# paulvoliva/XNODE-WAN-PDE-solver

Hardware: AMD Instinct MI355X
Metric: WAN training-steps/sec (optimiser sub-steps, d=20 cube, N_r=4096 paths per GPU) (higher is better)
Workload: dtype f64

## Files before the change

### include/xnwan.h

```cpp
#ifndef XNWAN_H
#define XNWAN_H
#ifdef __cplusplus
extern "C" {
#endif

#define XW_E_DIMS     (-1)
#define XW_E_ARG      (-2)
#define XW_E_WORKSPACE (-3)
#define XW_E_COMM     (-4)

int xw_abi_version(void);
int xw_supported_dims(char* buf, int buflen);

int xw_theta_size(int d, int H, int K);
int xw_phi_size(int d, int W);

int xw_ode_fwd(const double* xT, const double* t, const double* start, const double* theta,
               int method, int N, int L, int d, int H, int K, int m,
               double* u, double* Y, void* stream);

typedef struct { const double* xT; const double* start; double* u; double* Y; double* act; int N;
                 int act_x_only;
                 int narrow;
                 int prio_drop;
// ... 120 lines not shown
int xw_slab_sum(const double* gslab, int nslab, int P, int accumulate, double* out, void* stream);
int xw_slab_sum2(const double* gA, int nA, double* outA, const double* gB, int nB, double* outB, int P, void* stream);

typedef struct {
  int N, Nb, L, Lb, d;
  int same_grid;
  int w_per_point, amode, pair_i, pair_b;
  int ns_u, ns_b;
  int narrow;
  int sharded;
  double Vol, Nglob, Nbglob, s3_scale, init_off, bdry_off, ckappa;
  const double *xT, *xvT, *xbT, *t, *tb, *tpp, *xvT_pts;
  const double *start, *start_b, *h, *href, *f, *g, *w, *wt, *w0, *ghT, *gwx0T, *c, *cp, *A0, *B0;
  double *u, *ub, *Y, *Yb, *act, *act_b, *v, *vt, *gxv, *gtv, *gx, *gs, *vbar, *s3x, *vact, *slabA, *slabB, *slab_v, *work_i, *work_b;
  double *xproj;
} XwGroup;
typedef int (*XwExchangeFn)(double* buf, int count, void* ctx, void* stream);
typedef struct {
  int method, H, K, m, W, q, Pu, Pv, adjoint;
  int v_blocks, v_blocks_disc;
  int lag_lo, lag_hi;
  double alpha, pollution, lr_u, lr_v, beta1, beta2, eps;
  double *theta, *phi, *scal, *grad_u, *grad_v, *m_u, *v_u, *m_v, *v_v;
  long long *step_u, *step_v, *lag_u;
  XwExchangeFn exchange;
  void* exchange_ctx;
  double* pack_u;
  int merged_sweep;
} XwSolverState;
int xw_substep_gen(const XwGroup* g, const XwSolverState* s, int skip_v, int store_record, double* accum, int adam_skip_field,
// ... 27 lines not shown
```

### xnode_wan_pde_solver_amd/_lib.py

```python
import ctypes
import os

_HERE = os.path.dirname(os.path.abspath(__file__))
LIB_PATH = os.environ.get('XW_LIBRARY') or os.path.join(_HERE, 'libxnwan.so')
ABI_VERSION = 33

c_f32p = ctypes.c_void_p
c_f64p = ctypes.c_void_p
c_i64p = ctypes.c_void_p
c_int, c_dbl, c_vp = ctypes.c_int, ctypes.c_double, ctypes.c_void_p


class XwOdeFwdJob(ctypes.Structure):
    _fields_ = [('xT', c_vp), ('start', c_vp), ('u', c_vp), ('Y', c_vp), ('act', c_vp), ('N', c_int), ('act_x_only', c_int),
                ('narrow', c_int), ('prio_drop', c_int)]


class XwOdeBwdJob(ctypes.Structure):
    _fields_ = [('xT', c_vp), ('start', c_vp), ('Y', c_vp), ('act', c_vp), ('ubar', c_vp), ('gx', c_vp), ('gs', c_vp),
                ('gslab', c_vp), ('N', c_int), ('res_first_only', c_int), ('res_u', c_vp), ('res_ref', c_vp),
                ('res_coef', ctypes.c_double), ('res_base', ctypes.c_double), ('res_w_per_point', c_int), ('res_w', c_vp),
                ('res_c', c_vp), ('res_cp', c_vp), ('res_kappa2', ctypes.c_double), ('res_scal', c_vp), ('res_refA', c_vp),
                ('res_coefA', ctypes.c_double), ('res_baseA', ctypes.c_double)]

# ... 7 lines not shown
    _fields_ = [('xT', c_vp), ('start', c_vp), ('u', c_vp), ('Y', c_vp), ('rec_y', c_vp), ('rec_t', c_vp), ('rec_h', c_vp),
                ('fbuf', c_vp), ('ctl', c_vp), ('work', c_vp), ('N', c_int), ('cap', c_int)]


class XwDopriSweepJob(ctypes.Structure):
    _fields_ = [('b', XwOdeBwdJob), ('rec_y', c_vp), ('rec_t', c_vp), ('rec_h', c_vp), ('ctl', c_vp)]


class XwGroup(ctypes.Structure):
    _fields_ = ([(n, c_int) for n in ('N', 'Nb', 'L', 'Lb', 'd', 'same_grid', 'w_per_point', 'amode', 'pair_i', 'pair_b', 'ns_u', 'ns_b',
                                      'narrow', 'sharded')]
                + [(n, c_dbl) for n in ('Vol', 'Nglob', 'Nbglob', 's3_scale', 'init_off', 'bdry_off', 'ckappa')]
                + [(n, c_vp) for n in ('xT', 'xvT', 'xbT', 't', 'tb', 'tpp', 'xvT_pts', 'start', 'start_b', 'h', 'href', 'f', 'g', 'w',
                                       'wt', 'w0', 'ghT', 'gwx0T', 'c', 'cp', 'A0', 'B0', 'u', 'ub', 'Y', 'Yb', 'act', 'act_b', 'v',
                                       'vt', 'gxv', 'gtv', 'gx', 'gs', 'vbar', 's3x', 'vact', 'slabA', 'slabB', 'slab_v', 'work_i',
                                       'work_b', 'xproj')])


class XwSolverState(ctypes.Structure):
    _fields_ = ([(n, c_int) for n in ('method', 'H', 'K', 'm', 'W', 'q', 'Pu', 'Pv', 'adjoint', 'v_blocks', 'v_blocks_disc', 'lag_lo',
                                      'lag_hi')]
                + [(n, c_dbl) for n in ('alpha', 'pollution', 'lr_u', 'lr_v', 'beta1', 'beta2', 'eps')]
                + [(n, c_vp) for n in ('theta', 'phi', 'scal', 'grad_u', 'grad_v', 'm_u', 'v_u', 'm_v', 'v_v', 'step_u', 'step_v',
                                       'lag_u', 'exchange', 'exchange_ctx', 'pack_u')]
                + [('merged_sweep', c_int)])


EXCHANGE_FN = ctypes.CFUNCTYPE(ctypes.c_int, ctypes.c_void_p, ctypes.c_int, ctypes.c_void_p, ctypes.c_void_p)


SIGNATURES = {
# ... 124 lines not shown
```

### xnode_wan_pde_solver_amd/csrc/xw_disc.hip

```cpp
#include "xw_common.h"
#include "xw_generic.h"
#include <atomic>
#include <cstdlib>

namespace {

template <int W> struct VDim {
  static constexpr int MT = (W + 15) / 16;
  static constexpr int KS = (W + 3) / 4;
  static constexpr int TR = W - 16 * (MT - 1);
  static constexpr bool VTAIL = TR <= 3;
  static constexpr int MTF = VTAIL ? MT - 1 : MT;
  __device__ static constexpr int LR(int mt) { return (W + 1 - 16 * mt) >= 16 ? 4 : (W + 1 - 16 * mt + 3) / 4; }
  static constexpr bool BIASROW = (W % 16) != 0;
  static_assert(MT == 4 || MT == 6 || MT == 8, "row tiles of the compiled widths");
};

struct Pt {
  int p, n;
  bool valid;
  double t;
};
__device__ __forceinline__ Pt locate(long tile, long P, int N, const double* __restrict__ tf, const double* __restrict__ tpp) {
  Pt q;
// ... 106 lines not shown
  for (long it = (long)blockIdx.x * 4 + wave; it < ntiles;) {
    const long tile = DYN ? it : (it < G ? it - rot + (it < rot ? G : 0) : it);
    long nxt = it + G;
    unsigned int ticket = 0;
    if (DYN && lane == 0) ticket = atomicAdd(queue + cur * XW_DISC_QSTRIDE, 1u);
    const Pt pt = locate(tile, P, N, tf, tpp);
    const bool want_grad = gxv != nullptr && tile * 16 < ngrad;
    d4 a[D::MT], ad[D::MT];
    const long tu = __builtin_amdgcn_readfirstlane((int)tile);
    double* actl = act + tu * ((long)(q + 1) * W * 16);
    asm volatile("" : "+s"(actl));
    const int aoff = lane;
    const double* pht = ph;
    asm volatile("" : "+s"(pht));
    if (XPROJ) {
      const double* xp = xproj + pt.n;
#pragma unroll
      for (int mt = 0; mt < D::MT; ++mt)
#pragma unroll
        for (int r = 0; r < 4; ++r) {
          ad[mt][r] = sIn[16 * mt + g + 4 * r];
          a[mt][r] = (16 * mt + 4 * r < W) ? fma(ad[mt][r], pt.t, xw_ld_g(xp + (long)(16 * mt + 4 * r + g) * N)) : 0.0;
        }
    } else if (VINLDS) {
#pragma unroll
      for (int mt = 0; mt < D::MT; ++mt)
#pragma unroll
        for (int r = 0; r < 4; ++r) {
          ad[mt][r] = sIn[16 * mt + g + 4 * r];
          a[mt][r] = sIn[16 * D::MT + 16 * mt + g + 4 * r] + ad[mt][r] * pt.t;
        }
      for (int ks = 0; ks < ksl; ++ks) {
        const int i = 4 * ks + g;
        const double b = i < d ? xT[(long)i * N + pt.n] : 0.0;
#pragma unroll
        for (int mt = 0; mt < D::MT; ++mt) a[mt] = XW_MFMA(sVin[(ks * D::MT + mt) * 64 + lane], b, a[mt]);
      }
// ... 1129 lines not shown
```

### xnode_wan_pde_solver_amd/csrc/xw_substep.hip

```cpp
#include <hip/hip_runtime.h>
#include <string.h>
#include "xnwan.h"

namespace {
struct Side {
  hipStream_t s = nullptr;
  hipEvent_t fork = nullptr, fwd = nullptr, done = nullptr;
};
Side* side_of_current_device() {
  static Side sides[64];
  int dev = 0;
  if (hipGetDevice(&dev) != hipSuccess || dev < 0 || dev >= 64) return nullptr;
  Side& x = sides[dev];
  if (x.s == nullptr) {
    if (hipStreamCreateWithFlags(&x.s, hipStreamNonBlocking) != hipSuccess) return nullptr;
    if (hipEventCreateWithFlags(&x.fork, hipEventDisableTiming) != hipSuccess || hipEventCreateWithFlags(&x.fwd, hipEventDisableTiming) != hipSuccess ||
        hipEventCreateWithFlags(&x.done, hipEventDisableTiming) != hipSuccess)
      return nullptr;
  }
  return &x;
}
#define XW_HIP(call) { const hipError_t e_ = (call); if (e_ != hipSuccess) return (int)e_; }

inline XwOdeFwdJob fwd_job(const double* xT, const double* start, double* u, double* Y, double* act, int N, int x_only, int narrow) {
// ... 1 lines not shown
  j.xT = xT; j.start = start; j.u = u; j.Y = Y; j.act = act; j.N = N; j.act_x_only = x_only; j.narrow = narrow; j.prio_drop = 0;
  return j;
}
inline XwOdeBwdJob bwd_job(const double* xT, const double* start, const double* Y, const double* act, int N) {
  XwOdeBwdJob j;
  memset(&j, 0, sizeof(j));
  j.xT = xT; j.start = start; j.Y = Y; j.act = act; j.N = N;
  return j;
}
#define XW_TRY(call) { const int rc_ = (call); if (rc_ != 0) return rc_; }

int test_net(const XwGroup* g, const XwSolverState* s, int blocks, double* record, void* stream) {
  if (g->tpp != nullptr)
    return xw_disc_fwd(g->xvT_pts, nullptr, g->tpp, s->phi, g->N * g->L, 1, g->d, s->W, s->q, g->v, g->vt, g->gxv, g->gtv, g->N, blocks,
                       record, stream);
  if (g->xproj != nullptr) XW_TRY(xw_disc_xproj(g->xvT, s->phi, g->N, g->d, s->W, g->xproj, stream));
  return xw_disc_fwd_xproj(g->xvT, g->t, nullptr, s->phi, g->N, g->L, g->d, s->W, s->q, g->v, g->vt, g->gxv, g->gtv, g->N, blocks, record,
                           g->xproj, stream);
}
int contract(const XwGroup* g, const XwSolverState* s, long long* step, bool with_bdry, bool finalize, void* stream) {
  const double* s3x = nullptr;
  if (g->A0 != nullptr || g->B0 != nullptr) {
    XW_TRY(xw_weak_contract_general(g->A0, g->amode, g->B0, g->gx, g->gs, g->ghT, g->gxv, g->w0, g->gwx0T, g->v, g->d, g->N, g->s3x,
                                    stream));
    s3x = g->s3x;
  }
  const bool fused = s3x == nullptr;
  return xw_weak_partials(g->u, g->v, g->vt, g->w, g->w_per_point, g->wt, s3x, fused ? g->gx : nullptr, fused ? g->gs : nullptr,
                          fused ? g->ghT : nullptr, fused ? g->gxv : nullptr, fused ? g->w0 : nullptr, fused ? g->gwx0T : nullptr,
                          fused ? g->d : 0, g->c, g->ckappa, g->f, g->h, g->pair_i ? g->href : nullptr, g->pair_i ? 1 : 0,
                          g->pair_i ? g->s3_scale : 1.0, g->N, g->L, g->Vol, g->Nglob, g->work_i, s->scal, finalize ? 1 : 0,
// ... 189 lines not shown
      XW_TRY(xw_disc_bwd(g->xvT_pts, nullptr, g->tpp, s->phi, g->vbar, g->N * g->L, 1, g->d, s->W, s->q, record, g->slab_v, stream));
    } else {
      XW_TRY(xw_disc_bwd(g->xvT, g->t, nullptr, s->phi, g->vbar, g->N, g->L, g->d, s->W, s->q, record, g->slab_v, stream));
    }
  }
  if (!shard) {
    XW_TRY(xw_adam(s->phi, g->slab_v, nsv, accum, nullptr, 0, nullptr, nullptr, s->m_v, s->v_v, s->step_v, -1, s->Pv, s->lr_v, s->beta1,
                   s->beta2, s->eps, s->grad_v, 0, 0, 0, nullptr, stream));
  } else {
    if (have_i) { XW_TRY(xw_slab_sum(g->slab_v, nsv, s->Pv, 0, s->grad_v, stream)); } else { XW_ZERO(s->grad_v, s->Pv); }
    XW_TRY(s->exchange(s->grad_v, s->Pv, s->exchange_ctx, stream));
    XW_TRY(xw_losses(s->scal, g->L, g->Lb > 0 ? g->Lb : 1, g->Vol, g->Nglob, g->Nbglob, s->alpha, 0.0, 0.0, s->step_v, stream));
    XW_TRY(xw_adam(s->phi, accum, accum != nullptr ? 1 : 0, s->grad_v, nullptr, 0, nullptr, nullptr, s->m_v, s->v_v, s->step_v, -1, s->Pv,
                   s->lr_v, s->beta1, s->beta2, s->eps, s->grad_v, 0, 0, 0, nullptr, stream));
  }
  if (accum != nullptr) {
    const hipError_t e = hipMemcpyAsync(accum, s->grad_v, sizeof(double) * s->Pv, hipMemcpyDeviceToDevice, (hipStream_t)stream);
    if (e != hipSuccess) return (int)e;
  }
  return 0;
}
```

### xnode_wan_pde_solver_amd/engine.py

```python
import contextlib
import math
import os

import torch

from . import kernels as KN
from ._lib import XnwanError
from .options import EngineOptions
from .sampling import HIP_HOST_LOCK, _PIN_POOL, Hypercube, _paths


def ctypes_addr(fn):
    import ctypes
    return ctypes.cast(fn, ctypes.c_void_p).value

_KEPT_GRAPHS = []

_NOSTREAM = contextlib.nullcontext()

_SCRATCH_POOL = []


_DEVICE_STREAMS = {}

# ... 126 lines not shown
                                                                              KN.GENERIC_ODE_MAX_DEPTH, sorted(KN.METHODS)))
        self.testnet = getattr(v_mod, 'family', None) or KN.testnet_family(config['v_hidden_dim'], self.q)
        self.testnet_tiled = self.testnet == 'tiled'
        if self.testnet_tiled and self.W != config['v_hidden_dim']:
            raise XnwanError('the tiled test-network family reads phi at the network\'s own width; the module was bound at %d' % self.W)
        self.generic = (self.stepper == 'generic', not self.testnet_tiled and KN.disc_generic(self.W))
        if any(self.generic):
            import warnings
            which = ' and '.join(n_ for n_, g_ in zip(('u_theta (u_hidden_dim %d, u_hidden_hidden_dim %d, u_layers %d)' % (self.H, self.K, self.m),
                                                       'v_phi (v_hidden_dim %d)' % self.W), self.generic) if g_)
            warnings.warn('%s is outside the MFMA kernel instantiations %s (u_layers <= 10) / %s: running on the generic vector-ALU path, expect a step '
                          'rate lower by two to three orders of magnitude' % (which, KN.ODE_WIDTHS, KN.DISC_WIDTHS), RuntimeWarning, stacklevel=3)
        self.xproj_min_d = 1 << 30 if (self.generic[1] or self.testnet_tiled) else int(opt.xproj_min_d)
        if self.W > 64 and not self.generic[1] and not self.testnet_tiled:
            self.xproj_min_d = 0
        if self.generic[0] and self.adjoint:
            raise XnwanError('adjoint=True (the continuous adjoint) exists for the MFMA stepper instantiations %s only; u_hidden_dim = %d, '
                             'u_hidden_hidden_dim = %d run on the generic path, which reverses the steps taken (adjoint=False)'
                             % (KN.ODE_WIDTHS, self.H, self.K))
        self.theta, self.phi = u_mod.blob, v_mod.blob
        self.Pu, self.Pv = self.theta.data.numel(), self.phi.data.numel()
        z = lambda n: torch.zeros(n, dtype=F64, device=device)
        self.adam_u = dict(m=z(self.Pu), v=z(self.Pu), step=torch.zeros(1, dtype=torch.int64, device=device),
                           lag=torch.zeros(1, dtype=torch.int64, device=device))
        self.pairwise_single_slice = opt.pairwise_single_slice
        self.adam_skips_untouched = opt.adam_skips_untouched
        self.eager_checked = 10 ** 12 if opt.always_check else 256
        self.field_range = (self.theta.slots[6][0], self.theta.slots[-2][0])
        self._field_touched = False
        self.adam_v = dict(m=z(self.Pv), v=z(self.Pv), step=torch.zeros(1, dtype=torch.int64, device=device))
# ... 308 lines not shown
        pair_state = dict(pair_i=pair_i, pair_b=pair_b, init_off=init_off, bdry_off=bdry_off, s3_scale=nglob if pair_i else 1.0,
                          sharded=sharded, has_bdry=BX is not None and (nb_glob if sharded else Nb) > 0)
        if into is not None:
            G = into
            same = (G.N, G.L, G.Nb, G.Lb, G.same_grid, G.Vol, G.Nglob, G.Nbglob, G.pair_i, G.pair_b, G.amode, G.sharded) == (
                N, L, Nb, Lb, same_grid, vol, nglob, nbglob, pair_i, pair_b, amode, sharded) and all(
                (getattr(G, k) is None) == (S[k] is None) and (S[k] is None or getattr(G, k).shape == S[k].shape)
                for k in Group.SAMPLE_FIELDS)
            if same:
                for k in Group.SAMPLE_FIELDS:
                    if S[k] is not None:
                        getattr(G, k).copy_(S[k])
                G.domain = domain
                G.__dict__.update(pair_state)
                G.sample_version += 1
                return G
        G = Group()
        for k in Group.SAMPLE_FIELDS:
            setattr(G, k, S[k])
        G.domain, G.N, G.L, G.Nb, G.Vol, G.Nglob, G.Nbglob = domain, N, L, Nb, vol, nglob, nbglob
        G.Lb, G.same_grid, G.amode = Lb, same_grid, amode
        G.__dict__.update(pair_state)
        self._work_buffers(G, [])
        G.graphs = {}
        G.sample_version = into.sample_version + 1 if into is not None else 0
        return G

    def load_groups_packed(self, shards, hints, domain, cache, big):
        tc = getattr(self, '_tab_cat', None)
        st = self.structure
        if (tc is None or not (st.a_identity and st.b_zero and st.c_kappa is not None)
                or getattr(domain, 'time_independent', False) or any(h is None for h in hints)):
            return None
        srcs = [tc[k] for k in ('f', 'g', 'w', 'gw', 'start', 'gh', 'h', 'start_b')]
        if any(t.dtype != F64 or not t.is_cuda for t in srcs) or any(t.dtype != F64 or not t.is_cuda or t_[0] is not t_[1]
                                                                       for t_ in shards for t in t_[:3]):
            return None
        d, dev, T0 = self.d, self.dev, self.setup['T0']
        f_cat, g_cat, w_cat, gw_cat, start, gh, hv, sb = srcs
        if f_cat.stride(0) != 1 or g_cat.stride(0) != 1 or w_cat.stride(0) != 1:
# ... 6 lines not shown
        for k, ((X, XV, BX, n_glob, nb_glob, grids), hn) in enumerate(zip(shards, hints)):
            N, L, Nb, Lb = X.shape[0], X.shape[1], BX.shape[0], BX.shape[1]
            sharded = n_glob is not None and self.world is not None
            shared = bool(hn['shared_times'])
            same_grid = Lb == L and bool(hn['same_grid'])
            starts_T0, b_T0 = bool(tc['at0'][k]), bool(tc['bat0'][k])
            G = Group()
            G.domain, G.N, G.L, G.Nb, G.Vol = domain, N, L, Nb, vol
            G.Nglob, G.Nbglob = float(n_glob if n_glob is not None else N), float(nb_glob if nb_glob is not None else max(Nb, 1))
            G.Lb, G.same_grid, G.amode = Lb, same_grid, 0
            fields = [('t', (L,)), ('xT', (d, N))]
            if not shared:
                fields += [('tpp', (L * N,)), ('tpp0', (N,)), ('xvT_pts', (d, L * N))]
            fields += [('start', (N,)), ('ghT', (d, N)), ('h', (N,)), ('f', (L, N)), ('w', (L, N)), ('wt', (L, N)), ('w0', (N,)), ('gwx0T', (d, N)),
                       ('tb', (Lb,)), ('xbT', (d, Nb)), ('start_b', (Nb,)), ('g', (Lb, Nb))]
            self._work_buffers(G, fields)
            G._lazy['xvT'] = G._lazy['xT']
            if shared:
                G.tpp = G.tpp0 = G.xvT_pts = None
            G.href = G.X = G.A0 = G.B0 = None
            base = G._arena.data_ptr()
            x0, x1, x2 = X.stride()
            b0, b1, b2 = BX.stride()
            xp, bp = X.data_ptr(), BX.data_ptr()
            t_src = (xp, x1) if grids is None else (grids[0].data_ptr(), grids[0].stride(0))
            tb_src = (bp, b1) if grids is None else (grids[1].data_ptr(), grids[1].stride(0))
            src = {'t': (t_src[0], 1, 1, L, 0, 0, t_src[1]), 'xT': (xp + 8 * x2, 1, d, N, 0, x2, x0),
                   'tpp': (xp, 1, L, N, 0, x1, x0), 'tpp0': (xp, 1, 1, N, 0, 0, x0), 'xvT_pts': (xp + 8 * x2, d, L, N, x2, 0, x0),
                   'start': (start.data_ptr() + 8 * oN * start.stride(0), 1, 1, N, 0, 0, start.stride(0)),
                   'ghT': (gh.data_ptr() + 8 * oN * h0, 1, d, N, 0, h1, h0),
                   'h': (hv.data_ptr() + 8 * oN * hv.stride(0), 1, 1, N, 0, 0, hv.stride(0)),
# ... 22 lines not shown
            G.sample_version = ver + 1 if old is not None else 0
            if self.verify_structure and k == big and ver % self.verify_every == 0:
                self._check_structure(X, ver // self.verify_every)
            groups.append(G)
            oN, oNL, oNb, oNbL = oN + N, oNL + N * L, oNb + Nb, oNbL + Nb * Lb
        if len(rows) > KN.GATHER_ROWS:
            return None
        table = torch.zeros(KN.GATHER_ROWS, 9, dtype=torch.int64)
        table[:len(rows)] = torch.tensor(rows, dtype=torch.int64)
        from .sampling import _PIN_POOL
        pinned = _PIN_POOL.stage(table)
        tdev = pinned.to(dev, non_blocking=True)
        _PIN_POOL.uploaded(pinned, torch.cuda.current_stream(dev))
        KN.gather_fields(tdev, len(rows), total)
        for G in groups:
            if G.pair_i and not st.b_zero:
                raise XnwanError('func_b != 0 on a single-slice group at T0 (see load_group)')
            if G.pair_i or G.pair_b:
                zero = torch.zeros((), dtype=F64, device=dev)
                gsum, gsq = (G.g.sum(), (G.g ** 2).sum()) if G.pair_b else (zero, zero)
                stats = torch.stack([G.h.sum(), (G.h ** 2).sum(), G.f.sum(), gsum, gsq]).contiguous()
                if G.sharded:
                    self.world.all_reduce(stats)
                sh, shh, sf, sg, sgg = stats.tolist()
                if G.pair_i:
                    G.href = torch.full((G.N,), sh / G.Nglob, dtype=F64, device=dev)
                    G.f.fill_(sf / G.Nglob)
                    G.init_off = shh / G.Nglob - (sh / G.Nglob) ** 2
                if G.pair_b:
                    G.g.fill_(sg / G.Nbglob)
                    G.bdry_off = sgg / G.Nbglob - (sg / G.Nbglob) ** 2
        return groups

    def _work_buffers(self, G, fields):
        dev, d, N, L, Nb, Lb = self.dev, self.d, G.N, G.L, G.Nb, G.Lb
        poison = self.options.poison
        H = self.H
        ar = KN.ode_act_rows(self.method, H, self.K, self.m) if self.keep_activations and not self.adjoint else 0
        keep_v = self.keep_activations or self.testnet_tiled or not KN.disc_recompute(self.W, self.q)
        G.ns_u = KN.ode_bwd_slabs(N)
        G.ns_b = KN.ode_bwd_slabs(Nb) if Nb else 0
        nw = KN.reduce_work_size()
        plan = list(fields) + [('u', (L, N)), ('Y', (L, H, N)), ('v', (L, N)), ('vt', (L, N)), ('gxv', (d, N)), ('gtv', (N,)), ('gx', (d, N)), ('gs', (N,)),
                ('vbar', (L, N)), ('s3x', (N,)),
                ('slabA', (G.ns_u + G.ns_b, self.Pu)),
                ('slabB', (G.ns_u, self.Pu)),
                ('slab_v', (KN.disc_bwd_slabs(N, L), self.Pv)),
                ('work_i', (nw,)), ('work_b', (nw,))]
        if ar:
            plan.append(('act', (max(L - 1, 1), ar, KN.ode_act_cols(N))))
            if Nb:
                plan.append(('act_b', (max(Lb - 1, 1), ar, KN.ode_act_cols(Nb))))
        if keep_v:
            plan.append(('vact', (KN.disc_act_rows(self.W, self.q), KN.disc_act_cols(L * N))))
        if N and d >= self.xproj_min_d:
            plan.append(('xproj', (KN.disc_xproj_rows(self.W), N)))
        if Nb:
            plan += [('ub', (Lb, Nb)), ('Yb', (Lb, H, Nb))]
        lazy, off = {}, 0
        for name, shape in plan:
            lazy[name] = (off, shape)
            off += -(-math.prod(shape) // 64) * 64
        G._arena = torch.full((off,), float('nan'), dtype=F64, device=dev) if poison else torch.empty(off, dtype=F64, device=dev)
        G._lazy = lazy
        w0 = lazy['work_i'][0]
        G._arena[w0:lazy['work_b'][0] + nw].zero_()
        G.c = G.cp = None
        if not ar:
            G.act = G.act_b = None
        elif not Nb:
# ... 13 lines not shown
        t0 = float(times[0])
        td, du, dv, db = st
        ver = G.sample_version
        if self.verify_structure and ver % self.verify_every == 0:
            self._check_structure(_paths(td, du), ver // self.verify_every)

        lean = (self.structure.a_identity and self.structure.b_zero and self.structure.c_kappa is not None
                and getattr(domain, 'time_independent', False) and hasattr(domain, 'func_w_grad') and G.Nb > 0 and G.same_grid
                and not (G.pair_i or G.pair_b) and G.tpp is None
                and (G.N, G.L, G.Nb, G.Lb) == (du.shape[0], td.shape[0], db.shape[0], td.shape[0])
                and float(domain.V()) == G.Vol and n_glob in (None, G.Nglob) and nb_glob in (None, G.Nbglob))

        def body(_G):
            if lean:
                self._refill_fields(G, td, du, dv, db, domain, t0)
                return
            out = self.load_group(_paths(td, du), _paths(td, dv), _paths(td, db), domain, n_glob, nb_glob, into=G, shared_grid_t0=t0,
                                  verify=False)
            if out is not G:
                raise XnwanError('refill_compact: the sample does not have the shapes of the group it refills')
        key = 'refill_%r_%s_%r_%r_%r_%d_%r_%r' % (t0, type(domain).__name__, float(domain.V()), getattr(domain, 'top', None),
                                                  getattr(domain, 'bot', None), int(lean), n_glob, nb_glob)
        if key not in G.graphs and sum(1 for k in G.graphs if k.startswith('refill')) >= self.refill_variants:
            if not G.__dict__.get('_refill_cap_warned'):
                import warnings
                G._refill_cap_warned = True
                warnings.warn('more than %d variants of the refill graph for one group (first time / extent / path counts change from '
                              'sample to sample): further variants run as eager launches' % self.refill_variants, RuntimeWarning, stacklevel=2)
            G.graphs[key] = False
        self._run(G, key, body, scratch=True)
        G.domain, G.sample_version = domain, ver + 1
        return G

    def _refill_fields(self, G, td, du, dv, db, domain, t0):
        T0, fn = self.setup['T0'], self.funcs
        at0 = float(t0) == T0
        e0 = self._mark()
        with self._side(1, e0):
            X0 = _paths(td[:1], du)[:, 0, :].requires_grad_(True)
            s_ = fn['h'](X0) if at0 else fn['g'](X0.unsqueeze(1)).reshape(-1)
            G.start.copy_(s_.detach().reshape(-1))
            if s_.requires_grad:
                G.ghT.copy_(torch.autograd.grad(s_.sum(), X0)[0][:, 1:].t())
            else:
                G.ghT.zero_()
            G.h.copy_(G.start if at0 else fn['h'](X0.detach()).reshape(-1))
# ... 36 lines not shown

    def _join(self, *events):
        if self.use_streams:
            cur = torch.cuda.current_stream()
            for ev in events:
                if ev is not None:
                    cur.wait_event(ev)

    def _launch_test_net_here(self, G, blocks=None):
        ph, blocks = self.phi.data, blocks or self.v_blocks
        act = G.vact if getattr(G, 'vact_valid', False) else None
        if G.tpp is not None:
            KN.disc_fwd(G.xvT_pts, None, ph, self.W, self.q, tpp=G.tpp, v=G.v.view(1, -1), vt=G.vt.view(1, -1),
                        gxv=G.gxv, gtv=G.gtv, ngrad=G.N, max_blocks=blocks, act=act)
        else:
            xp = KN.disc_xproj(G.xvT, ph, self.W, out=G.xproj) if 'xproj' in G._lazy else None
            KN.disc_fwd(G.xvT, G.t, ph, self.W, self.q, v=G.v, vt=G.vt, gxv=G.gxv, gtv=G.gtv, ngrad=G.N,
                        max_blocks=blocks, act=act, xproj=xp)

    def _reaction(self, G):
        ck = self.structure.c_kappa
        if ck is None and G.pair_i:
            N = G.N
            ul = G.u.t().detach().requires_grad_(True)
            with torch.enable_grad():
                c = self.funcs['c'](G.X, ul)
                c = c.reshape(N, N) if c.numel() == N * N and N > 1 else c.reshape(-1)
                if c.dim() == 2:
                    if getattr(G, 'sharded', False):
                        raise XnwanError('func_c returns a table over all pairs of paths on a single-slice group (it mixes u [N, 1] with a slice of X that '
                                         'kept its last axis): that needs every path of the group on one rank -- run such groups replicated '
# ... 77 lines not shown
                      'xproj', 'slabA', 'slabB', 'slab_v', 'work_i', 'work_b', 'ub', 'Yb'):
                setattr(xg, k, G.ptr(k))
            nar = lambda jobs, **kw: self._narrow_ok(jobs, **kw)
            ji, jb = self._job(G, 'i'), (self._job(G, 'b') if G.Nb else None)
            joint = G.Nb and G.same_grid
            bits = [nar([ji] + ([jb] if joint else []), alone=False, forward=True),
                    bool(jb) and nar([jb], alone=False, forward=True),
                    nar([ji] + ([jb] if joint else []) + [ji], alone=False),
                    bool(jb) and nar([jb], alone=False),
                    bool(joint) and nar([ji, jb], alone=False),
                    nar([ji], alone=False, params=False),
                    nar([ji], alone=False, forward=True),
                    nar([ji], alone=False, params=False)]
            xg.narrow = sum(1 << i for i, b in enumerate(bits) if b)
        xg.sharded = int(bool(getattr(G, 'sharded', False)))
        xg.pair_i, xg.pair_b = int(bool(G.pair_i)), int(bool(G.pair_b))
        xg.Vol, xg.Nglob, xg.Nbglob, xg.s3_scale = float(G.Vol), float(G.Nglob), float(G.Nbglob), float(G.s3_scale)
        xg.init_off, xg.bdry_off, xg.ckappa = float(G.init_off), float(G.bdry_off), float(self.structure.c_kappa)
        xg.href = 0 if G.href is None else G.href.data_ptr()
        xg.c = xg.cp = 0
        return xg

    def _runner_ok(self, G):
        return (self.use_runner and self.structure.c_kappa is not None and G.c is None and not getattr(G, 'persistent', True))

    def _world_of(self, G):
        return self.world if getattr(G, 'sharded', self.world is not None) else None

    def _field_seen(self, G):
        touched = G.L > 1 or (getattr(G, 'has_bdry', G.Nb > 0) and G.Lb > 1)
# ... 189 lines not shown
        elif world is None and getattr(G, 'sumA_ready', False) and acc is None:
            KN.adam(self.theta.data, None, st['m'], st['v'], st['step'], lr, gslabB=G.slabB, scal=self.scal,
                    gextraA=G.sumA, gsum_out=self.grad_u, bump_step=-1, **lag)
        elif world is None:
            KN.adam(self.theta.data, G.slabA, st['m'], st['v'], st['step'], lr, gslabB=G.slabB, scal=self.scal,
                    gextraA=acc, gsum_out=self.grad_u, bump_step=-1, **lag)
        else:
            P = self.Pu
            if acc is not None:
                self.pack_u[:P].add_(acc)
            KN.adam(self.theta.data, None, st['m'], st['v'], st['step'], lr, gextraA=self.pack_u[:P],
                    gextraB=self.pack_u[P:2 * P], scal=self.scal, gsum_out=self.grad_u, bump_step=-1, **lag)
        if acc is not None:
            acc.copy_(self.grad_u)

    def _v_fresh(self, G, store=False):
        now = self._v_key(G)
        G.skip_v = self.reuse_test_net and getattr(G, 'v_version', None) == now
        G.v_version = now
        if not G.skip_v:
            G.vact_valid = G.vact is not None and (store or self.reuse_test_net)
        return ('_vcached' if G.skip_v else '') + ('_act' if getattr(G, 'vact_valid', False) else '')

    def _v_key(self, G):
        return (self._phi_version, sum(p._version for p in self.phi.params), G.sample_version)

    def invalidate_test_net(self):
        self._phi_version += 1

    def _run_runner(self, fn, *args):
        from ._lib import check
        self._exchange_error = None
        rc = fn(*args)
        if getattr(self, '_exchange_error', None) is not None:
            err, self._exchange_error = self._exchange_error, None
            raise err
        check(rc, fn.__name__)

    def generator_step(self, G):
        sfx = self._v_fresh(G)
        world = self._world_of(G)
        if self._runner_ok(G):
            from ._lib import lib
            skip = self.adam_skips_untouched and not self._field_seen(G)
            G.ck = self.structure.c_kappa
            self._run_runner(lib.xw_substep_gen, self._runner_group(G), self._runner_state(), int(bool(G.skip_v)),
                             int(bool(getattr(G, 'vact_valid', False))), KN._p(self.accum_u), int(skip), KN._stream())
            return
        if world is None:
            self._run(G, 'gen' + sfx, self._gen_all)
            return
        if self.capture_exchange:
            self._run(G, 'gen_dist' + sfx, self._gen_all_dist)
            return
# ... 67 lines not shown
        KN.slab_sum(G.slab_v, out=self.grad_v)

    def _disc_back(self, G):
        lr, st = self.config['v_rate'], self.adam_v
        acc = self.accum_v
        world = self._world_of(G)
        if world is not None:
            KN.losses(self.scal, G.L, G.Lb, G.Vol, G.Nglob, G.Nbglob, self.alpha, step=st['step'])
        if world is None:
            KN.adam(self.phi.data, G.slab_v, st['m'], st['v'], st['step'], lr, gextraA=acc, gsum_out=self.grad_v,
                    bump_step=-1)
        else:
            if acc is not None:
                self.grad_v.add_(acc)
            KN.adam(self.phi.data, None, st['m'], st['v'], st['step'], lr, gextraA=self.grad_v, bump_step=-1)
        if acc is not None:
            acc.copy_(self.grad_v)

    def _reduce_sums(self, G):
        self.world.all_reduce(self.scal[0:9])
        if G.pair_i:
            KN.pair_fold(self.scal, G.Vol, G.Nglob)

    def _disc_all(self, G):
        self._disc_front(G)
        self._disc_mid(G)
        self._disc_back(G)

    def _disc_all_dist(self, G):
        self._disc_front(G)
        self._reduce_sums(G)
        self._disc_mid_packed(G)
        self.world.all_reduce(self.grad_v)
        self._disc_back(G)

    def discriminator_step(self, G):
        sfx = self._v_fresh(G, store=True)
        self._phi_version += 1
        world = self._world_of(G)
        if self._runner_ok(G):
            from ._lib import lib
            G.ck = self.structure.c_kappa
            self._run_runner(lib.xw_substep_disc, self._runner_group(G), self._runner_state(), int(bool(G.skip_v)),
                             int(bool(getattr(G, 'vact_valid', False))), KN._p(self.accum_v), KN._stream())
            return
        if world is None:
            self._run(G, 'disc' + sfx, self._disc_all)
            return
        if self.capture_exchange:
            self._run(G, 'disc_dist' + sfx, self._disc_all_dist)
            return
        self._run(G, 'disc_front' + sfx, self._disc_front)
        self._reduce_sums(G)
# ... 129 lines not shown
```

### xnode_wan_pde_solver_amd/options.py

```python
import dataclasses
import os
from typing import Optional


def _flag(name, default):
    v = os.environ.get(name)
    if v is None:
        return default
    return v != '0' if default else v == '1'


def _int(name, default):
    v = os.environ.get(name)
    return default if v in (None, '') else int(v)


@dataclasses.dataclass
class EngineOptions:
    use_streams: bool = True
    use_graphs: bool = True
    strict_graphs: bool = False
    reuse_test_net: bool = False
    keep_activations: bool = True
    v_blocks: int = 0
    v_blocks_disc: int = 0
    narrow: str = '1'
    narrow_set: str = 'fx'
    narrow_tiles: Optional[str] = None
    narrow_tiles_alone: str = '256:256:64'
    early_slab_sum: bool = True
    merged_sweep: bool = True
    compact_tiles: int = 320
    prio_drop_A: Optional[int] = None
    prio_drop_X: int = 0
    prio_drop_F: int = 0
    prio_drop_G: int = 0
    use_runner: bool = True
    capture_exchange: bool = True
    xproj_min_d: int = 45
    tiled_stepper: str = 'beyond'
    eval_chunk_paths: int = 65536
    hw_queues: int = 4
    verify_structure: bool = True
    packed_load: bool = True
    pairwise_single_slice: bool = True
    adam_skips_untouched: bool = True
    always_check: bool = False
    poison: bool = False
    capture_refill: bool = True
    defer_list_readback: bool = True
    sampler_process: bool = True
    show_plan: bool = False
    dopri5_chunk: int = 8
    dopri5_max_steps: int = 10000
# ... 13 lines not shown
        o.v_blocks_disc = _int('XW_V_BLOCKS_DISC', o.v_blocks_disc)
        o.narrow = os.environ.get('XW_NARROW', o.narrow)
        o.narrow_set = os.environ.get('XW_NARROW_SET', o.narrow_set)
        o.narrow_tiles = os.environ.get('XW_NARROW_TILES') or None
        o.narrow_tiles_alone = os.environ.get('XW_NARROW_TILES_ALONE') or o.narrow_tiles_alone
        o.early_slab_sum = _flag('XW_EARLY_SLAB_SUM', o.early_slab_sum)
        o.merged_sweep = _flag('XW_MERGED_SWEEP', o.merged_sweep)
        o.compact_tiles = _int('XW_COMPACT_TILES', o.compact_tiles)
        o.prio_drop_A = _int('XW_PRIO_DROP_A', None)
        o.prio_drop_X = _int('XW_PRIO_DROP_X', o.prio_drop_X)
        o.prio_drop_F = _int('XW_PRIO_DROP_F', o.prio_drop_F)
        o.prio_drop_G = _int('XW_PRIO_DROP_G', o.prio_drop_G)
        o.use_runner = _flag('XW_RUNNER', o.use_runner)
        o.capture_exchange = _flag('XW_CAPTURE_EXCHANGE', o.capture_exchange)
        o.xproj_min_d = _int('XW_XPROJ_MIN_D', o.xproj_min_d)
        o.tiled_stepper = os.environ.get('XW_TILED_STEPPER') or o.tiled_stepper
        o.eval_chunk_paths = _int('XW_EVAL_CHUNK_PATHS', o.eval_chunk_paths)
        try:
            o.hw_queues = _int('GPU_MAX_HW_QUEUES', o.hw_queues)
        except ValueError:
            pass
        o.verify_structure = _flag('XW_VERIFY_STRUCTURE', o.verify_structure)
        o.packed_load = _flag('XW_PACKED_LOAD', o.packed_load)
        o.pairwise_single_slice = not _flag('XW_ELEMENTWISE_SINGLE_SLICE', False)
        o.adam_skips_untouched = not _flag('XW_ADAM_NO_SKIP', False)
        o.always_check = _flag('XW_ALWAYS_CHECK', o.always_check)
        o.poison = _flag('XW_POISON', o.poison)
        o.capture_refill = _flag('XW_CAPTURE_REFILL', o.capture_refill)
        o.defer_list_readback = _flag('XW_DEFER_LIST', o.defer_list_readback)
        o.sampler_process = _flag('XW_SAMPLER_PROCESS', o.sampler_process)
# ... 12 lines not shown
```

### xnode_wan_pde_solver_amd/solver.py

```python
import json
import os
import time
from itertools import product

import torch

from . import nets, sampling
from .sampling import HIP_HOST_LOCK
from ._lib import XnwanError
from .engine import Engine
from .options import EngineOptions
from .kernels import adam as _adam_kernel

CONFIG_KEYS = ['alpha', 'u_layers', 'u_hidden_dim', 'u_hidden_hidden_dim', 'v_layers', 'v_hidden_dim', 'n1', 'n2',
               'u_rate', 'v_rate', 'min_steps', 'adjoint', 'solver']
SETUP_KEYS = ['dim', 'N_t', 'N_r', 'N_b', 'T0', 'T', 'shape_param']


def split_params(params):
    missing = [k for k in CONFIG_KEYS + SETUP_KEYS[:-1] + ['iterations', 'domain'] if k not in params]
    if missing:
        raise KeyError('params is missing %s' % missing)
    config = {k: params[k] for k in CONFIG_KEYS}
    setup = {k: params[k] for k in SETUP_KEYS if k in params}
# ... 351 lines not shown
            'refill': 'one graph replay per sample' if (cube and self.capture_refill and eng.use_graphs and not self.tabulate_on_host) else
                      ('one packed upload + one gather launch per sample' if (not cube and eng.packed_load and not self.tabulate_on_host) else 'group by group'),
            'sub_steps': 'captured HIP graphs' if (cube and eng.use_graphs) else ('one C call per group sub-step (xw_substep_*)' if eng.use_runner and
                                                                                 eng.structure.c_kappa is not None else 'launch by launch'),
            'ode_solver': ("dopri5 (adaptive, step sizes chosen on the device per group; its sub-steps run as eager launches, "
                           "controllers read back every %d attempts; dopri5_stepper = '%s': %s)"
                           % (self.options.dopri5_chunk, eng.dopri5_stepper,
                              'the field on the tiled MFMA stepper, csrc/xw_tdopri.hip' if eng.dopri5_stepper == 'tiled' else
                              'the field per path on the vector ALU, csrc/xw_dopri.hip') if eng.dopri5 else
                           '%s (fixed grid: the sample times%s)' % (self.config['solver'], ', Adams-Bashforth AB3 .. AB11 after two rk4 '
                                                                     'start-up steps' if self.config['solver'] == 'explicit_adams' else '')),
            'stepper': {'mfma': 'fused MFMA container %s' % ((eng.H, eng.K),), 'generic': 'generic vector-ALU path (csrc/xw_generic.hip)',
                        'tiled': 'tiled MFMA family (csrc/xw_tiled.hip)'}[eng.stepper],
            'testnet': ('tiled MFMA family at width %d (csrc/xw_disc_tiled.hip)' % eng.W if eng.testnet == 'tiled' else
                        'generic vector-ALU path (csrc/xw_generic.hip)' if eng.generic[1] else 'fused MFMA container %d' % eng.W),
            'ranks': 1 if self.world is None else self.world.size,
            'exchange': None if self.world is None else ('xw_allreduce (RCCL) on the stream: inside the sub-step graphs / the group runner'
                                                         if self.world.capturable else 'torch.distributed, staged through the host'),
            'small_groups': None if (self.world is None or cube) else ('replicated below %d paths per rank' % self.world.replicate_below
                                                                       if self.world.replicate_below > 0 else 'sharded (empty shares)'),
            'test_net_reuse_inside_an_outer_iteration': bool(self.reuse_test_net),
            'coefficients': eng.structure.describe(),
            'options_not_at_their_defaults': self.options.non_default(),
        }

    def train(self, report=False, report_it=10, show_plt=False):
        if self.options.show_plan and self._is_main():
            print('train() plan: ' + json.dumps(self.plan(report)))
        threads = torch.get_num_threads()
        if self.host_threads:
# ... 510 lines not shown
```

Measured before the change: 2166.

## Cache the test network's x-projection table across sub-steps and enable it from d=20

Keeps a per-path table of the test network's input-layer projection (phi applied to x). The table is formed when a sample is loaded and right after the discriminator's Adam update, and is reused at the head of test-network launches when phi and the sample are unchanged. This lowers the table threshold so d=20 now uses it, which removes the per-point input matmul and the repeated per-launch projection. The cost is extra memory, version-key bookkeeping, graph key variants, and staleness risk if a phi change goes undetected. The kernel's indexing of the table was also adjusted to put the row offset into a scalar register.

```diff
diff --git a/include/xnwan.h b/include/xnwan.h
--- a/include/xnwan.h
+++ b/include/xnwan.h
@@ -158,6 +158,7 @@
   const double *start, *start_b, *h, *href, *f, *g, *w, *wt, *w0, *ghT, *gwx0T, *c, *cp, *A0, *B0;
   double *u, *ub, *Y, *Yb, *act, *act_b, *v, *vt, *gxv, *gtv, *gx, *gs, *vbar, *s3x, *vact, *slabA, *slabB, *slab_v, *work_i, *work_b;
   double *xproj;
+  int xproj_current;
 } XwGroup;
 typedef int (*XwExchangeFn)(double* buf, int count, void* ctx, void* stream);
 typedef struct {
diff --git a/xnode_wan_pde_solver_amd/_lib.py b/xnode_wan_pde_solver_amd/_lib.py
--- a/xnode_wan_pde_solver_amd/_lib.py
+++ b/xnode_wan_pde_solver_amd/_lib.py
@@ -45,7 +45,8 @@
                 + [(n, c_vp) for n in ('xT', 'xvT', 'xbT', 't', 'tb', 'tpp', 'xvT_pts', 'start', 'start_b', 'h', 'href', 'f', 'g', 'w',
                                        'wt', 'w0', 'ghT', 'gwx0T', 'c', 'cp', 'A0', 'B0', 'u', 'ub', 'Y', 'Yb', 'act', 'act_b', 'v',
                                        'vt', 'gxv', 'gtv', 'gx', 'gs', 'vbar', 's3x', 'vact', 'slabA', 'slabB', 'slab_v', 'work_i',
-                                       'work_b', 'xproj')])
+                                       'work_b', 'xproj')]
+                + [('xproj_current', c_int)])
 
 
 class XwSolverState(ctypes.Structure):
diff --git a/xnode_wan_pde_solver_amd/csrc/xw_disc.hip b/xnode_wan_pde_solver_amd/csrc/xw_disc.hip
--- a/xnode_wan_pde_solver_amd/csrc/xw_disc.hip
+++ b/xnode_wan_pde_solver_amd/csrc/xw_disc.hip
@@ -144,13 +144,15 @@
     const double* pht = ph;
     asm volatile("" : "+s"(pht));
     if (XPROJ) {
-      const double* xp = xproj + pt.n;
+      int Nl = N;
+      asm volatile("" : "+s"(Nl));
+      const double* xp = xproj + pt.n + (long)g * Nl;
 #pragma unroll
       for (int mt = 0; mt < D::MT; ++mt)
 #pragma unroll
         for (int r = 0; r < 4; ++r) {
           ad[mt][r] = sIn[16 * mt + g + 4 * r];
-          a[mt][r] = (16 * mt + 4 * r < W) ? fma(ad[mt][r], pt.t, xw_ld_g(xp + (long)(16 * mt + 4 * r + g) * N)) : 0.0;
+          a[mt][r] = (16 * mt + 4 * r < W) ? fma(ad[mt][r], pt.t, xw_ld_g(xp + (long)(16 * mt + 4 * r) * Nl)) : 0.0;
         }
     } else if (VINLDS) {
 #pragma unroll
diff --git a/xnode_wan_pde_solver_amd/csrc/xw_substep.hip b/xnode_wan_pde_solver_amd/csrc/xw_substep.hip
--- a/xnode_wan_pde_solver_amd/csrc/xw_substep.hip
+++ b/xnode_wan_pde_solver_amd/csrc/xw_substep.hip
@@ -39,7 +39,7 @@
   if (g->tpp != nullptr)
     return xw_disc_fwd(g->xvT_pts, nullptr, g->tpp, s->phi, g->N * g->L, 1, g->d, s->W, s->q, g->v, g->vt, g->gxv, g->gtv, g->N, blocks,
                        record, stream);
-  if (g->xproj != nullptr) XW_TRY(xw_disc_xproj(g->xvT, s->phi, g->N, g->d, s->W, g->xproj, stream));
+  if (g->xproj != nullptr && g->xproj_current != 2) XW_TRY(xw_disc_xproj(g->xvT, s->phi, g->N, g->d, s->W, g->xproj, stream));
   return xw_disc_fwd_xproj(g->xvT, g->t, nullptr, s->phi, g->N, g->L, g->d, s->W, s->q, g->v, g->vt, g->gxv, g->gtv, g->N, blocks, record,
                            g->xproj, stream);
 }
@@ -259,6 +259,8 @@
     XW_TRY(xw_adam(s->phi, accum, accum != nullptr ? 1 : 0, s->grad_v, nullptr, 0, nullptr, nullptr, s->m_v, s->v_v, s->step_v, -1, s->Pv,
                    s->lr_v, s->beta1, s->beta2, s->eps, s->grad_v, 0, 0, 0, nullptr, stream));
   }
+  if (have_i && g->xproj != nullptr && g->tpp == nullptr && g->xproj_current != 0 && accum == nullptr)
+    XW_TRY(xw_disc_xproj(g->xvT, s->phi, g->N, g->d, s->W, g->xproj, stream));
   if (accum != nullptr) {
     const hipError_t e = hipMemcpyAsync(accum, s->grad_v, sizeof(double) * s->Pv, hipMemcpyDeviceToDevice, (hipStream_t)stream);
     if (e != hipSuccess) return (int)e;
diff --git a/xnode_wan_pde_solver_amd/engine.py b/xnode_wan_pde_solver_amd/engine.py
--- a/xnode_wan_pde_solver_amd/engine.py
+++ b/xnode_wan_pde_solver_amd/engine.py
@@ -164,6 +164,8 @@
         self.xproj_min_d = 1 << 30 if (self.generic[1] or self.testnet_tiled) else int(opt.xproj_min_d)
         if self.W > 64 and not self.generic[1] and not self.testnet_tiled:
             self.xproj_min_d = 0
+        self.xproj_cached = bool(opt.xproj_cached) and self.xproj_min_d < (1 << 30)
+        self.xproj_table_min_d = min(self.xproj_min_d, int(opt.xproj_cached_min_d)) if self.xproj_cached else self.xproj_min_d
         if self.generic[0] and self.adjoint:
             raise XnwanError('adjoint=True (the continuous adjoint) exists for the MFMA stepper instantiations %s only; u_hidden_dim = %d, '
                              'u_hidden_hidden_dim = %d run on the generic path, which reverses the steps taken (adjoint=False)'
@@ -502,6 +504,7 @@
                 G.domain = domain
                 G.__dict__.update(pair_state)
                 G.sample_version += 1
+                self._form_xproj(G)
                 return G
         G = Group()
         for k in Group.SAMPLE_FIELDS:
@@ -512,6 +515,7 @@
         self._work_buffers(G, [])
         G.graphs = {}
         G.sample_version = into.sample_version + 1 if into is not None else 0
+        self._form_xproj(G)
         return G
 
     def load_groups_packed(self, shards, hints, domain, cache, big):
@@ -548,7 +552,7 @@
                 fields += [('tpp', (L * N,)), ('tpp0', (N,)), ('xvT_pts', (d, L * N))]
             fields += [('start', (N,)), ('ghT', (d, N)), ('h', (N,)), ('f', (L, N)), ('w', (L, N)), ('wt', (L, N)), ('w0', (N,)), ('gwx0T', (d, N)),
                        ('tb', (Lb,)), ('xbT', (d, Nb)), ('start_b', (Nb,)), ('g', (Lb, Nb))]
-            self._work_buffers(G, fields)
+            self._work_buffers(G, fields, cached_table=False)
             G._lazy['xvT'] = G._lazy['xT']
             if shared:
                 G.tpp = G.tpp0 = G.xvT_pts = None
@@ -601,6 +605,8 @@
         _PIN_POOL.uploaded(pinned, torch.cuda.current_stream(dev))
         KN.gather_fields(tdev, len(rows), total)
         for G in groups:
+            self._form_xproj(G)
+        for G in groups:
             if G.pair_i and not st.b_zero:
                 raise XnwanError('func_b != 0 on a single-slice group at T0 (see load_group)')
             if G.pair_i or G.pair_b:
@@ -619,7 +625,7 @@
                     G.bdry_off = sgg / G.Nbglob - (sg / G.Nbglob) ** 2
         return groups
 
-    def _work_buffers(self, G, fields):
+    def _work_buffers(self, G, fields, cached_table=True):
         dev, d, N, L, Nb, Lb = self.dev, self.d, G.N, G.L, G.Nb, G.Lb
         poison = self.options.poison
         H = self.H
@@ -640,7 +646,8 @@
                 plan.append(('act_b', (max(Lb - 1, 1), ar, KN.ode_act_cols(Nb))))
         if keep_v:
             plan.append(('vact', (KN.disc_act_rows(self.W, self.q), KN.disc_act_cols(L * N))))
-        if N and d >= self.xproj_min_d:
+        point_mode = G.__dict__.get('tpp') is not None or any(n_ == 'tpp' for n_, _ in fields)
+        if N and (d >= self.xproj_min_d or (cached_table and d >= self.xproj_table_min_d and not point_mode)):
             plan.append(('xproj', (KN.disc_xproj_rows(self.W), N)))
         if Nb:
             plan += [('ub', (Lb, Nb)), ('Yb', (Lb, H, Nb))]
@@ -684,6 +691,7 @@
         def body(_G):
             if lean:
                 self._refill_fields(G, td, du, dv, db, domain, t0)
+                self._form_xproj(G)
                 return
             out = self.load_group(_paths(td, du), _paths(td, dv), _paths(td, db), domain, n_glob, nb_glob, into=G, shared_grid_t0=t0,
                                   verify=False)
@@ -700,6 +708,8 @@
             G.graphs[key] = False
         self._run(G, key, body, scratch=True)
         G.domain, G.sample_version = domain, ver + 1
+        if self._xproj_held(G):
+            G.xproj_key = self._v_key(G)
         return G
 
     def _refill_fields(self, G, td, du, dv, db, domain, t0):
@@ -766,7 +776,9 @@
             KN.disc_fwd(G.xvT_pts, None, ph, self.W, self.q, tpp=G.tpp, v=G.v.view(1, -1), vt=G.vt.view(1, -1),
                         gxv=G.gxv, gtv=G.gtv, ngrad=G.N, max_blocks=blocks, act=act)
         else:
-            xp = KN.disc_xproj(G.xvT, ph, self.W, out=G.xproj) if 'xproj' in G._lazy else None
+            xp = None
+            if 'xproj' in G._lazy:
+                xp = G.xproj if getattr(G, 'xproj_cur', False) else KN.disc_xproj(G.xvT, ph, self.W, out=G.xproj)
             KN.disc_fwd(G.xvT, G.t, ph, self.W, self.q, v=G.v, vt=G.vt, gxv=G.gxv, gtv=G.gtv, ngrad=G.N,
                         max_blocks=blocks, act=act, xproj=xp)
 
@@ -874,6 +886,7 @@
                     nar([ji], alone=False, params=False)]
             xg.narrow = sum(1 << i for i, b in enumerate(bits) if b)
         xg.sharded = int(bool(getattr(G, 'sharded', False)))
+        xg.xproj_current = (2 if getattr(G, 'xproj_cur', False) else 1) if self._xproj_held(G) else 0
         xg.pair_i, xg.pair_b = int(bool(G.pair_i)), int(bool(G.pair_b))
         xg.Vol, xg.Nglob, xg.Nbglob, xg.s3_scale = float(G.Vol), float(G.Nglob), float(G.Nbglob), float(G.s3_scale)
         xg.init_off, xg.bdry_off, xg.ckappa = float(G.init_off), float(G.bdry_off), float(self.structure.c_kappa)
@@ -1093,13 +1106,42 @@
         if acc is not None:
             acc.copy_(self.grad_u)
 
+    def xproj_plan(self):
+        if self.xproj_min_d >= (1 << 30):
+            return 'per point (the %s test-network family has no x-projection table)' % ('tiled' if self.testnet_tiled else 'generic')
+        if self.d < self.xproj_table_min_d:
+            return 'per point (d = %d: the x-projection table is used from d = %d on)' % (self.d, self.xproj_table_min_d)
+        if self.xproj_cached:
+            return ('x-projection table per path, cached (from d = %d on): formed where the sample is loaded and behind the '
+                    'discriminator\'s update, at the head of a launch only when phi or the sample changed otherwise' % self.xproj_table_min_d)
+        return 'x-projection table per path, formed at the head of every test-network launch (from d = %d on)' % self.xproj_table_min_d
+
+    def _xproj_held(self, G):
+        return self.xproj_cached and G.N > 0 and G.tpp is None and 'xproj' in G._lazy
+
+    def _form_xproj(self, G):
+        if self._xproj_held(G):
+            KN.disc_xproj(G.xvT, self.phi.data, self.W, out=G.xproj)
+            G.xproj_key = self._v_key(G)
+
+    def _xproj_tail(self, G):
+        return self._xproj_held(G) and self.accum_v is None
+
+    def _xproj_state(self, G, now):
+        G.xproj_cur = False
+        if G.skip_v or not self._xproj_held(G):
+            return ''
+        G.xproj_cur = getattr(G, 'xproj_key', None) == now
+        G.xproj_key = now
+        return '_xc' if G.xproj_cur else ''
+
     def _v_fresh(self, G, store=False):
         now = self._v_key(G)
         G.skip_v = self.reuse_test_net and getattr(G, 'v_version', None) == now
         G.v_version = now
         if not G.skip_v:
             G.vact_valid = G.vact is not None and (store or self.reuse_test_net)
-        return ('_vcached' if G.skip_v else '') + ('_act' if getattr(G, 'vact_valid', False) else '')
+        return ('_vcached' if G.skip_v else '') + ('_act' if getattr(G, 'vact_valid', False) else '') + self._xproj_state(G, now)
 
     def _v_key(self, G):
         return (self._phi_version, sum(p._version for p in self.phi.params), G.sample_version)
@@ -1117,6 +1159,15 @@
         check(rc, fn.__name__)
 
     def generator_step(self, G):
+        try:
+            self._generator_step(G)
+        except BaseException:
+            G.xproj_key = None
+            raise
+        finally:
+            G.xproj_cur = False
+
+    def _generator_step(self, G):
         sfx = self._v_fresh(G)
         world = self._world_of(G)
         if self._runner_ok(G):
@@ -1214,6 +1265,8 @@
             if acc is not None:
                 self.grad_v.add_(acc)
             KN.adam(self.phi.data, None, st['m'], st['v'], st['step'], lr, gextraA=self.grad_v, bump_step=-1)
+        if self._xproj_tail(G):
+            KN.disc_xproj(G.xvT, self.phi.data, self.W, out=G.xproj)
         if acc is not None:
             acc.copy_(self.grad_v)
 
@@ -1235,8 +1288,23 @@
         self._disc_back(G)
 
     def discriminator_step(self, G):
+        try:
+            self._discriminator_step(G)
+        except BaseException:
+            G.xproj_key = None
+            raise
+        finally:
+            G.xproj_cur = False
+
+    def _disc_bookkeeping(self, G):
         sfx = self._v_fresh(G, store=True)
         self._phi_version += 1
+        if self._xproj_tail(G):
+            G.xproj_key = self._v_key(G)
+        return sfx
+
+    def _discriminator_step(self, G):
+        sfx = self._disc_bookkeeping(G)
         world = self._world_of(G)
         if self._runner_ok(G):
             from ._lib import lib
diff --git a/xnode_wan_pde_solver_amd/options.py b/xnode_wan_pde_solver_amd/options.py
--- a/xnode_wan_pde_solver_amd/options.py
+++ b/xnode_wan_pde_solver_amd/options.py
@@ -38,6 +38,8 @@
     use_runner: bool = True
     capture_exchange: bool = True
     xproj_min_d: int = 45
+    xproj_cached: bool = True
+    xproj_cached_min_d: int = 20
     tiled_stepper: str = 'beyond'
     eval_chunk_paths: int = 65536
     hw_queues: int = 4
@@ -81,6 +83,8 @@
         o.use_runner = _flag('XW_RUNNER', o.use_runner)
         o.capture_exchange = _flag('XW_CAPTURE_EXCHANGE', o.capture_exchange)
         o.xproj_min_d = _int('XW_XPROJ_MIN_D', o.xproj_min_d)
+        o.xproj_cached = _flag('XW_XPROJ_CACHED', o.xproj_cached)
+        o.xproj_cached_min_d = _int('XW_XPROJ_CACHED_MIN_D', o.xproj_cached_min_d)
         o.tiled_stepper = os.environ.get('XW_TILED_STEPPER') or o.tiled_stepper
         o.eval_chunk_paths = _int('XW_EVAL_CHUNK_PATHS', o.eval_chunk_paths)
         try:
diff --git a/xnode_wan_pde_solver_amd/solver.py b/xnode_wan_pde_solver_amd/solver.py
--- a/xnode_wan_pde_solver_amd/solver.py
+++ b/xnode_wan_pde_solver_amd/solver.py
@@ -389,6 +389,7 @@
                         'tiled': 'tiled MFMA family (csrc/xw_tiled.hip)'}[eng.stepper],
             'testnet': ('tiled MFMA family at width %d (csrc/xw_disc_tiled.hip)' % eng.W if eng.testnet == 'tiled' else
                         'generic vector-ALU path (csrc/xw_generic.hip)' if eng.generic[1] else 'fused MFMA container %d' % eng.W),
+            'testnet_input_layer': eng.xproj_plan(),
             'ranks': 1 if self.world is None else self.world.size,
             'exchange': None if self.world is None else ('xw_allreduce (RCCL) on the stream: inside the sub-step graphs / the group runner'
                                                          if self.world.capturable else 'torch.distributed, staged through the host'),
```

Measured after the change: 2199, median of 6. +1.5%, better.
